# ShuangXieIrene/ssds.pytorch

Measured on AMD Instinct MI355X. Metric: images/sec (fwd+decode+NMS) SSD-MobileNetV2@512, higher is better.
Workload: dtype bf16

## Files before the change

ssds.pytorch_amd/csrc/ssdk_mbk.hip:

```cpp
#include "ssdk_common.h"
#include "ssdk_flow_common.h"
#include "ssdk_scan.h"

namespace ssdk {

struct MbkParams {
  const u16* x;
  u16* y;
  const unsigned char* img;
  int N, H, W, Ho, Wo, Cin, Chid, Cout, residual;
  int pairs, halves;
  unsigned items;
  unsigned long long* dbg;
  unsigned wave_mask, pair_mask;
};

template <int KS, int NW, int NCHW, int NFO>
struct MbkGeo {
  static constexpr int NP = (NCHW + 1) / 2;
  static constexpr int PAIR_KB = 2 * KS + NFO;
  static constexpr int MISC_KB = (NCHW * 384 + 1023) / 1024;
  static constexpr int m_be = 0, m_wd = NCHW * 64, m_bd = NCHW * (64 + 288);
  static constexpr int SPB_KB = 2;
  static_assert(NFO * 128 <= SPB_KB * 1024, "projection BN block");
  __host__ __device__ static size_t weights(int halves) { return (size_t)halves * NW * NP * PAIR_KB * 1024; }
  __host__ __device__ static size_t misc_off(int halves) { return weights(halves); }
  __host__ __device__ static size_t spb_off(int halves) { return misc_off(halves) + (size_t)NW * MISC_KB * 1024; }
  __host__ __device__ static size_t bytes(int halves) { return spb_off(halves) + (size_t)halves * SPB_KB * 1024; }
};

template <int S, int NS>
struct MbkItem {
  static constexpr int NXS = NS * S;
  static constexpr int NR = S + 3;
};

template <int S, int NS, int KS, int NW, int NCHW, int NFO>
struct MbkLds {
  using G = MbkGeo<KS, NW, NCHW, NFO>;
  using I = MbkItem<S, NS>;
  static constexpr int FT = 2 * NS * NFO;
  static constexpr int XF = FT % 5 == 0 ? 5 : (FT % 8 == 0 ? 8 : 4);
  static_assert(FT % XF == 0, "exchange rounds");
  static constexpr int xt = 0;
  static constexpr int misc = xt + I::NR * I::NXS * KS * 1024;
  static constexpr int spb = misc + NW * G::MISC_KB * 1024;
  static constexpr int xch = spb + G::SPB_KB * 1024;
  static constexpr int bytes = xch + NW * XF * 1024;
};

__device__ __forceinline__ void mbk_mfma_guard() {
  __builtin_amdgcn_sched_barrier(0);
  asm volatile("s_nop 15\n\ts_nop 3" ::: "memory");
  __builtin_amdgcn_sched_barrier(0);
}
__device__ __forceinline__ void mbk_valu_guard() {
  __builtin_amdgcn_sched_barrier(0);
  asm volatile("s_nop 3" ::: "memory");
  __builtin_amdgcn_sched_barrier(0);
}
__device__ __forceinline__ u32 fl_from_left2(u32 cur, u32 prev) {
  const int old = __builtin_amdgcn_update_dpp(0, (int)prev, 0x121, 0xf, 0xf, true);
  return (u32)__builtin_amdgcn_update_dpp(old, (int)cur, 0x111, 0xf, 0xf, false);
}
__device__ __forceinline__ u32 fl_from_right2(u32 cur, u32 next) {
  const int old = __builtin_amdgcn_update_dpp(0, (int)next, 0x12f, 0xf, 0xf, true);
  return (u32)__builtin_amdgcn_update_dpp(old, (int)cur, 0x101, 0xf, 0xf, false);
}

template <int DT, int S, int NS, int KS, int NW, int NCHW, int NFO, bool DBG = false>
__global__ __launch_bounds__(64 * NW, 2) void mbk_kernel(const MbkParams p) {
  using L = MbkLds<S, NS, KS, NW, NCHW, NFO>;
  using G = MbkGeo<KS, NW, NCHW, NFO>;
  using I = MbkItem<S, NS>;
  constexpr int NR = I::NR, NXS = I::NXS, NE = NR * NXS;
  constexpr int XF = L::XF, FT = L::FT, NP = G::NP, PAIR_KB = G::PAIR_KB;
  constexpr int NO = 2 * NS;
  constexpr bool ODD = (NCHW & 1) != 0;
  constexpr int ROUNDS = FT / XF;
  extern __shared__ __attribute__((aligned(16))) unsigned char smem[];
  const u32 tid = threadIdx.x, lane = tid & 63u;
  const u32 fr = lane & 15u, fg = lane >> 4;
  const int wv = __builtin_amdgcn_readfirstlane((int)(tid >> 6));
  const int Cin = p.Cin, Cout = p.Cout, H = p.H, W = p.W, Ho = p.Ho, Wo = p.Wo;

  const u32 item = blockIdx.x;
  const int half = (int)(item % (u32)p.halves);
  const u32 rem = item / (u32)p.halves;
  const int n = (int)(rem / (u32)p.pairs), rp = (int)(rem % (u32)p.pairs);
  const int oy0 = 2 * rp;
  const int iy0 = S * oy0 - 1;
  const int co_base = half * 16 * NFO;
  const u16* ximg = p.x + (size_t)n * H * W * Cin;
  const bool stamp = p.dbg != nullptr && blockIdx.x == 0 && tid == 0;
  if (stamp) p.dbg[0] = __builtin_readcyclecounter();

  const u32x4* wimg = reinterpret_cast<const u32x4*>(p.img + ((size_t)(half * NW + wv) * NP) * ((size_t)PAIR_KB * 1024)) + lane;
  u32x4 wa[KS], wb[KS];
#pragma unroll
  for (int ks = 0; ks < KS; ++ks) {
    wa[ks] = wimg[(size_t)ks * 64];
    wb[ks] = wimg[(size_t)(KS + ks) * 64];
  }

  for (int e = wv; e < NE; e += NW) {
    const int r = e / NXS, xs = e % NXS;
    int iy = iy0 + r;
    iy = iy < 0 ? 0 : (iy > H - 1 ? H - 1 : iy);
    const int col = S == 1 ? 16 * xs + (int)fr : 2 * (16 * (xs >> 1) + (int)fr) + (xs & 1);
    const u16* src = ximg + ((size_t)iy * W + col) * Cin + fg * 8;
#pragma unroll
    for (int ks = 0; ks < KS; ++ks)
      __builtin_amdgcn_global_load_lds((glb_u8*)(src + ks * 32), (lds_u8*)(smem + L::xt + (e * KS + ks) * 1024), 16, 0, 0);
  }
  {
    const unsigned char* src = p.img + G::misc_off(p.halves) + (size_t)wv * (G::MISC_KB * 1024) + lane * 16;
#pragma unroll
    for (int k = 0; k < G::MISC_KB; ++k)
      __builtin_amdgcn_global_load_lds((glb_u8*)(src + k * 1024), (lds_u8*)(smem + L::misc + (wv * G::MISC_KB + k) * 1024), 16, 0, 0);
  }
  if (wv == 0) {
    const unsigned char* src = p.img + G::spb_off(p.halves) + (size_t)half * (G::SPB_KB * 1024) + lane * 16;
#pragma unroll
    for (int k = 0; k < G::SPB_KB; ++k)
      __builtin_amdgcn_global_load_lds((glb_u8*)(src + k * 1024), (lds_u8*)(smem + L::spb + k * 1024), 16, 0, 0);
  }
  asm volatile("s_waitcnt vmcnt(0)" ::: "memory");
  __syncthreads();
  if (stamp) p.dbg[1] = __builtin_readcyclecounter();

  fl_f2 hi[NR];
#pragma unroll
  for (int r = 0; r < NR; ++r) {
    const float k = ((unsigned)(iy0 + r) < (unsigned)H) ? kFlSixth : 0.f;
    hi[r] = fl_f2{k, k};
  }

  f32x4 yacc[NO][NFO];
#pragma unroll
  for (int o = 0; o < NO; ++o)
#pragma unroll
    for (int f = 0; f < NFO; ++f) yacc[o][f] = f32x4{0.f, 0.f, 0.f, 0.f};

  const unsigned char* xt = smem + L::xt + lane * 16;
  const unsigned char* mc = smem + L::misc + wv * (G::MISC_KB * 1024);

  auto chunk = [&](int c, const u32x4 (&w)[KS], u32 (&dout)[NO][2]) {
    const f32x4 bv = *reinterpret_cast<const f32x4*>(mc + G::m_be + (c * 4 + (int)fg) * 16);
    f32x4 e[NE];
#pragma unroll
    for (int i = 0; i < NE; ++i) e[i] = bv;
#pragma unroll
    for (int ks = 0; ks < KS; ++ks) {
      u32x4 xf[NE];
#pragma unroll
      for (int i = 0; i < NE; ++i) xf[i] = *reinterpret_cast<const u32x4*>(xt + (i * KS + ks) * 1024);
#pragma unroll
      for (int i = 0; i < NE; ++i) e[i] = fl_mfma<DT>(w[ks], xf[i], e[i]);
    }
    uint2 wt[9];
#pragma unroll
    for (int t = 0; t < 9; ++t) wt[t] = *reinterpret_cast<const uint2*>(mc + G::m_wd + ((c * 9 + t) * 4 + (int)fg) * 8);
    const uint2 bdi = *reinterpret_cast<const uint2*>(mc + G::m_bd + (c * 4 + (int)fg) * 8);
    mbk_mfma_guard();
    u32 ew[NR][NXS][2];
#pragma unroll
    for (int r = 0; r < NR; ++r)
#pragma unroll
      for (int xs = 0; xs < NXS; ++xs) {
        ew[r][xs][0] = fl_unit_pack(e[r * NXS + xs][0], e[r * NXS + xs][1], hi[r]);
        ew[r][xs][1] = fl_unit_pack(e[r * NXS + xs][2], e[r * NXS + xs][3], hi[r]);
      }
#pragma unroll
    for (int o = 0; o < 2; ++o)
#pragma unroll
      for (int j = 0; j < NS; ++j) {
        fl_h2 s[2] = {fl_as_h2(bdi.x), fl_as_h2(bdi.y)};
#pragma unroll
        for (int ky = 0; ky < 3; ++ky) {
          const int r = S * o + ky;
          const uint2 w0 = wt[ky * 3], w1 = wt[ky * 3 + 1], w2 = wt[ky * 3 + 2];
#pragma unroll
          for (int wd = 0; wd < 2; ++wd) {
            u32 tl, tc, tr;
            if constexpr (S == 1) {
              tc = ew[r][j][wd];
              tl = j == 0 ? fl_from_left(tc) : fl_from_left2(tc, ew[r][j > 0 ? j - 1 : 0][wd]);
              tr = j == NS - 1 ? fl_from_right(tc) : fl_from_right2(tc, ew[r][j < NS - 1 ? j + 1 : j][wd]);
            } else {
              const u32 odd = ew[r][2 * j + 1][wd];
              tc = ew[r][2 * j][wd];
              tl = j == 0 ? fl_from_left(odd) : fl_from_left2(odd, ew[r][j > 0 ? 2 * j - 1 : 1][wd]);
              tr = odd;
            }
            const u32 ww0 = wd ? w0.y : w0.x, ww1 = wd ? w1.y : w1.x, ww2 = wd ? w2.y : w2.x;
            s[wd] = __builtin_elementwise_fma(fl_as_h2(tl), fl_as_h2(ww0), s[wd]);
            s[wd] = __builtin_elementwise_fma(fl_as_h2(tc), fl_as_h2(ww1), s[wd]);
            if (ky == 2) s[wd] = fl_fma_clamp01(fl_as_h2(tr), fl_as_h2(ww2), s[wd]);
            else s[wd] = __builtin_elementwise_fma(fl_as_h2(tr), fl_as_h2(ww2), s[wd]);
          }
        }
        dout[o * NS + j][0] = fl_as_u32(s[0]);
        dout[o * NS + j][1] = fl_as_u32(s[1]);
      }
  };

  constexpr int FH = NFO / 2;
  for (int t = 0; t < NP; ++t) {
    const u32x4* wp = wimg + (size_t)t * (PAIR_KB * 64);
    const bool last = t == NP - 1;
    const u32x4* wn = wimg + (size_t)(last ? t : t + 1) * (PAIR_KB * 64);
    u32 d0[NO][2], d1[NO][2];
    u32x4 wf0[FH], wf1[NFO - FH];
#pragma unroll
    for (int f = 0; f < FH; ++f) wf0[f] = wp[(size_t)(2 * KS + f) * 64];
    chunk(2 * t, wa, d0);
    __builtin_amdgcn_sched_barrier(0);
    u32x4 na[KS];
#pragma unroll
    for (int ks = 0; ks < KS; ++ks) na[ks] = wn[(size_t)ks * 64];
#pragma unroll
    for (int f = FH; f < NFO; ++f) wf1[f - FH] = wp[(size_t)(2 * KS + f) * 64];
    if (!(ODD && last)) {
      chunk(2 * t + 1, wb, d1);
    } else {
#pragma unroll
      for (int o = 0; o < NO; ++o) d1[o][0] = d1[o][1] = 0u;
    }
    __builtin_amdgcn_sched_barrier(0);
    u32x4 nb[KS];
#pragma unroll
    for (int ks = 0; ks < KS; ++ks) nb[ks] = wn[(size_t)(KS + ks) * 64];
    u32x4 db[NO];
#pragma unroll
    for (int o = 0; o < NO; ++o) db[o] = u32x4{d0[o][0], d0[o][1], d1[o][0], d1[o][1]};
    if constexpr (DBG) {
      if (!((p.pair_mask >> t) & 1u) || !((p.wave_mask >> wv) & 1u)) {
#pragma unroll
        for (int o = 0; o < NO; ++o) db[o] = u32x4{0u, 0u, 0u, 0u};
      }
    }
    mbk_valu_guard();
#pragma unroll
    for (int f = 0; f < NFO; ++f)
#pragma unroll
      for (int o = 0; o < NO; ++o)
        yacc[o][f] = fl_mfma<SSDK_F16>(f < FH ? wf0[f < FH ? f : 0] : wf1[f >= FH ? f - FH : 0], db[o], yacc[o][f]);
    __builtin_amdgcn_sched_barrier(0);
#pragma unroll
    for (int ks = 0; ks < KS; ++ks) {
      wa[ks] = na[ks];
      wb[ks] = nb[ks];
    }
  }
  if (stamp) p.dbg[2] = __builtin_readcyclecounter();

  unsigned char* xb = smem + L::xch;
  const unsigned char* spb = smem + L::spb;
  constexpr int GPW = (XF + NW - 1) / NW;
  uint2 resv[ROUNDS][GPW];
#pragma unroll
  for (int R = 0; R < ROUNDS; ++R)
#pragma unroll
    for (int gg = 0; gg < GPW; ++gg) {
      const int g = wv + gg * NW, q = R * XF + g, oj = q / NFO, f = q % NFO;
      const int oy = oy0 + oj / NS, ox = 16 * (oj % NS) + (int)fr, co = co_base + f * 16 + (int)fg * 4;
      resv[R][gg] = make_uint2(0u, 0u);
      if (S == 1 && p.residual && g < XF && oy < Ho && co < Cout)
        resv[R][gg] = *reinterpret_cast<const uint2*>(ximg + ((size_t)oy * W + ox) * Cin + co);
    }
#pragma unroll
  for (int R = 0; R < ROUNDS; ++R) {
#pragma unroll
    for (int g = 0; g < XF; ++g) {
      const int q = R * XF + g, oj = q / NFO, f = q % NFO;
      *reinterpret_cast<f32x4*>(xb + ((wv * XF + g) * 64 + (int)lane) * 16) = yacc[oj][f];
    }
    __syncthreads();
#pragma unroll
    for (int gg = 0; gg < GPW; ++gg) {
      const int g = wv + gg * NW;
      if (g < XF) {
        const int q = R * XF + g, oj = q / NFO, f = q % NFO;
        f32x4 y = *reinterpret_cast<const f32x4*>(xb + ((0 * XF + g) * 64 + (int)lane) * 16);
#pragma unroll
        for (int w2 = 1; w2 < NW; ++w2) {
          const f32x4 t2 = *reinterpret_cast<const f32x4*>(xb + ((w2 * XF + g) * 64 + (int)lane) * 16);
          y = y + t2;
        }
        const int oy = oy0 + oj / NS, ox = 16 * (oj % NS) + (int)fr;
        const int co = co_base + f * 16 + (int)fg * 4;
        if (oy < Ho && co < Cout) {
          const f32x4 spv = *reinterpret_cast<const f32x4*>(spb + (f * 4 + (int)fg) * 32);
          const f32x4 bpv = *reinterpret_cast<const f32x4*>(spb + (f * 4 + (int)fg) * 32 + 16);
          u32 h01 = fl_pack2<DT>(fmaf(y[0], spv[0], bpv[0]), fmaf(y[1], spv[1], bpv[1]));
          u32 h23 = fl_pack2<DT>(fmaf(y[2], spv[2], bpv[2]), fmaf(y[3], spv[3], bpv[3]));
          if (S == 1 && p.residual) {
            const uint2 xr = resv[R][gg];
            h01 = fl_pack2<DT>(fl_from16<DT>(h01 & 0xffffu) + fl_from16<DT>(xr.x & 0xffffu), fl_from16<DT>(h01 >> 16) + fl_from16<DT>(xr.x >> 16));
            h23 = fl_pack2<DT>(fl_from16<DT>(h23 & 0xffffu) + fl_from16<DT>(xr.y & 0xffffu), fl_from16<DT>(h23 >> 16) + fl_from16<DT>(xr.y >> 16));
          }
          u16* yrow = p.y + (((size_t)n * Ho + oy) * Wo + ox) * Cout;
          *reinterpret_cast<uint2*>(yrow + co) = make_uint2(h01, h23);
        }
      }
    }
    if (R + 1 < ROUNDS) __syncthreads();
  }
  if (stamp) p.dbg[3] = __builtin_readcyclecounter();
}

template <int DT, int S, int NS, int KS, int NW, int NCHW, int NFO, bool DBG = false>
static void mbk_launch(const MbkParams& p, hipStream_t stream) {
  constexpr int lds = MbkLds<S, NS, KS, NW, NCHW, NFO>::bytes;
  static_assert(lds <= 160 * 1024, "LDS");
  (void)hipFuncSetAttribute(reinterpret_cast<const void*>(&mbk_kernel<DT, S, NS, KS, NW, NCHW, NFO, DBG>),
                            hipFuncAttributeMaxDynamicSharedMemorySize, lds);
  hipLaunchKernelGGL((mbk_kernel<DT, S, NS, KS, NW, NCHW, NFO, DBG>), dim3(p.items), dim3(64 * NW), lds, stream, p);
}

constexpr int kMbkNW = 4;
struct MbkInst {
  int s, ns, ks, nchw, nfo;
};
static const MbkInst kMbkInst[] = {{1, 1, 5, 15, 10}, {2, 1, 3, 9, 10}, {1, 2, 2, 6, 4}, {1, 2, 2, 6, 6}, {1, 2, 3, 9, 6},
                                   {2, 2, 1, 3, 4}, {1, 4, 1, 3, 2}};

static int mbk_find(int stride, int Wo, int Cin, int Chid, int Cout, int nw, int* halves) {
  if (nw != kMbkNW || Cin % 32 || Chid % 16 || Cout % 16 || Wo % 16) return -1;
  const int ks = Cin / 32, nch = Chid / 16, nchw = (nch + nw - 1) / nw, ns = Wo / 16;
  for (int i = 0; i < (int)(sizeof(kMbkInst) / sizeof(kMbkInst[0])); ++i) {
    const MbkInst& k = kMbkInst[i];
    if (k.s == stride && k.ns == ns && k.ks == ks && k.nchw == nchw && Cout % (16 * k.nfo) == 0) {
      if (halves) *halves = Cout / (16 * k.nfo);
      return i;
    }
  }
  return -1;
}

static size_t mbk_bytes(int inst, int halves) {
  switch (inst) {
    case 0: return MbkGeo<5, kMbkNW, 15, 10>::bytes(halves);
    case 1: return MbkGeo<3, kMbkNW, 9, 10>::bytes(halves);
    case 2: return MbkGeo<2, kMbkNW, 6, 4>::bytes(halves);
    case 3: return MbkGeo<2, kMbkNW, 6, 6>::bytes(halves);
    case 4: return MbkGeo<3, kMbkNW, 9, 6>::bytes(halves);
    case 5: return MbkGeo<1, kMbkNW, 3, 4>::bytes(halves);
    case 6: return MbkGeo<1, kMbkNW, 3, 2>::bytes(halves);
  }
  return 0;
}

template <int DT>
static void mbk_dispatch(const MbkParams& p, int inst, hipStream_t stream) {
  const bool dbg = p.wave_mask != ~0u || p.pair_mask != ~0u;
  switch (inst) {
    case 0: dbg ? mbk_launch<DT, 1, 1, 5, kMbkNW, 15, 10, true>(p, stream) : mbk_launch<DT, 1, 1, 5, kMbkNW, 15, 10>(p, stream); break;
    case 1: mbk_launch<DT, 2, 1, 3, kMbkNW, 9, 10>(p, stream); break;
    case 2: mbk_launch<DT, 1, 2, 2, kMbkNW, 6, 4>(p, stream); break;
    case 3: mbk_launch<DT, 1, 2, 2, kMbkNW, 6, 6>(p, stream); break;
    case 4: mbk_launch<DT, 1, 2, 3, kMbkNW, 9, 6>(p, stream); break;
    case 5: mbk_launch<DT, 2, 2, 1, kMbkNW, 3, 4>(p, stream); break;
    case 6: mbk_launch<DT, 1, 4, 1, kMbkNW, 3, 2>(p, stream); break;
  }
}

int launch_mbk(const ssdk_mbconv_desc* d, hipStream_t stream) {
  static const int env = getenv("SSDK_MBK") ? atoi(getenv("SSDK_MBK")) : 1;
  const int variant = d->variant;
  if ((!env && variant != 3) || (variant != 0 && variant != 3)) return 1;
  if (d->stem || !d->w_image || d->image_nw < 1 || (d->stride != 1 && d->stride != 2)) return 1;
  const int Ho = (d->H + 2 - 3) / d->stride + 1, Wo = (d->W + 2 - 3) / d->stride + 1;
  if (d->W != Wo * d->stride) return 1;
  int halves = 0;
  const int inst = mbk_find(d->stride, Wo, d->Cin, d->Chid, d->Cout, d->image_nw, &halves);
  if (inst < 0 || (size_t)d->w_image_bytes < mbk_bytes(inst, halves) || ((uintptr_t)d->w_image & 15)) return 1;
  if (env != 1 && variant != 3 && !((env >> (inst + 1)) & 1)) return 1;
  const int pairs = (Ho + 1) / 2;
  const long items = (long)halves * d->N * pairs;
  constexpr int env_min = 256;
  if (items < env_min && variant != 3) return 1;
  MbkParams p;
  p.x = (const u16*)d->x;
  p.y = (u16*)d->y;
  p.img = (const unsigned char*)d->w_image;
  p.N = d->N;
  p.H = d->H;
  p.W = d->W;
  p.Ho = Ho;
  p.Wo = Wo;
  p.Cin = d->Cin;
  p.Chid = d->Chid;
  p.Cout = d->Cout;
  p.residual = d->residual;
  p.pairs = pairs;
  p.halves = halves;
  p.items = (unsigned)items;
  p.dbg = nullptr;
  p.wave_mask = p.pair_mask = ~0u;
  if (const char* m = getenv("SSDK_MBK_MASKS")) {
    unsigned a = ~0u, b = ~0u;
    if (sscanf(m, "%x,%x", &a, &b) == 2) {
      p.wave_mask = a;
      p.pair_mask = b;
    }
  }
  static const int env_dbg = getenv("SSDK_MB_DBG") ? atoi(getenv("SSDK_MB_DBG")) : 0;
  static unsigned long long* dbg_dev = nullptr;
  if (env_dbg) {
    if (!dbg_dev) (void)hipMalloc(&dbg_dev, 8 * sizeof(unsigned long long));
    p.dbg = dbg_dev;
  }
  if (d->dtype == SSDK_BF16) mbk_dispatch<SSDK_BF16>(p, inst, stream);
  else mbk_dispatch<SSDK_F16>(p, inst, stream);
  if (env_dbg) {
    unsigned long long h[4];
    (void)hipStreamSynchronize(stream);
    (void)hipMemcpy(h, dbg_dev, sizeof(h), hipMemcpyDeviceToHost);
    fprintf(stderr, "[mbk dbg] Cin=%d Chid=%d Cout=%d s=%d W=%d items=%ld : setup %llu loop %llu exchange %llu\n", d->Cin, d->Chid,
            d->Cout, d->stride, d->W, items, h[1] - h[0], h[2] - h[1], h[3] - h[2]);
  }
  return 0;
}

}

extern "C" size_t ssdk_mbk_image_bytes(int Cin, int Chid, int Cout, int stride, int Wo, int nw, int* nfo) {
  int halves = 0;
  const int inst = ssdk::mbk_find(stride, Wo, Cin, Chid, Cout, nw, &halves);
  if (inst < 0) return 0;
  if (nfo) *nfo = ssdk::kMbkInst[inst].nfo;
  return ssdk::mbk_bytes(inst, halves);
}
```

Baseline: 64660.

## Process four output rows per block for the first MBConv instance

Generalises the fused MBConv kernel from two output rows per work item to a template parameter R, and sets R=4 for instance 0 (stride 1, KS=5, 15 hidden chunks per wave). Each block now loads a taller input halo (3R+... rows) once, so the weight image and halo rows are amortised over more outputs and fewer blocks are launched. For R=4 the input tile is also preloaded into registers once instead of re-read from LDS for every hidden chunk. In exchange, register pressure rises sharply, occupancy drops to one block per SIMD via launch bounds, and the number of blocks is halved, which could hurt latency hiding and load balance.

```diff
diff --git a/ssds.pytorch_amd/csrc/ssdk_mbk.hip b/ssds.pytorch_amd/csrc/ssdk_mbk.hip
--- a/ssds.pytorch_amd/csrc/ssdk_mbk.hip
+++ b/ssds.pytorch_amd/csrc/ssdk_mbk.hip
@@ -9,7 +9,7 @@
   u16* y;
   const unsigned char* img;
   int N, H, W, Ho, Wo, Cin, Chid, Cout, residual;
-  int pairs, halves;
+  int groups, halves;
   unsigned items;
   unsigned long long* dbg;
   unsigned wave_mask, pair_mask;
@@ -29,18 +29,19 @@
   __host__ __device__ static size_t bytes(int halves) { return spb_off(halves) + (size_t)halves * SPB_KB * 1024; }
 };
 
-template <int S, int NS>
+template <int S, int NS, int R>
 struct MbkItem {
+  static_assert(R == 2 || R == 4, "rows per item");
   static constexpr int NXS = NS * S;
-  static constexpr int NR = S + 3;
+  static constexpr int NR = S * (R - 1) + 3;
 };
 
-template <int S, int NS, int KS, int NW, int NCHW, int NFO>
+template <int S, int NS, int KS, int NW, int NCHW, int NFO, int R>
 struct MbkLds {
   using G = MbkGeo<KS, NW, NCHW, NFO>;
-  using I = MbkItem<S, NS>;
-  static constexpr int FT = 2 * NS * NFO;
-  static constexpr int XF = FT % 5 == 0 ? 5 : (FT % 8 == 0 ? 8 : 4);
+  using I = MbkItem<S, NS, R>;
+  static constexpr int FT = R * NS * NFO;
+  static constexpr int XF = FT % 8 == 0 ? 8 : (FT % 5 == 0 ? 5 : 4);
   static_assert(FT % XF == 0, "exchange rounds");
   static constexpr int xt = 0;
   static constexpr int misc = xt + I::NR * I::NXS * KS * 1024;
@@ -68,14 +69,14 @@
   return (u32)__builtin_amdgcn_update_dpp(old, (int)cur, 0x101, 0xf, 0xf, false);
 }
 
-template <int DT, int S, int NS, int KS, int NW, int NCHW, int NFO, bool DBG = false>
-__global__ __launch_bounds__(64 * NW, 2) void mbk_kernel(const MbkParams p) {
-  using L = MbkLds<S, NS, KS, NW, NCHW, NFO>;
+template <int DT, int S, int NS, int KS, int NW, int NCHW, int NFO, int R, bool DBG = false>
+__global__ __launch_bounds__(64 * NW, R == 2 ? 2 : 1) void mbk_kernel(const MbkParams p) {
+  using L = MbkLds<S, NS, KS, NW, NCHW, NFO, R>;
   using G = MbkGeo<KS, NW, NCHW, NFO>;
-  using I = MbkItem<S, NS>;
+  using I = MbkItem<S, NS, R>;
   constexpr int NR = I::NR, NXS = I::NXS, NE = NR * NXS;
   constexpr int XF = L::XF, FT = L::FT, NP = G::NP, PAIR_KB = G::PAIR_KB;
-  constexpr int NO = 2 * NS;
+  constexpr int NO = R * NS;
   constexpr bool ODD = (NCHW & 1) != 0;
   constexpr int ROUNDS = FT / XF;
   extern __shared__ __attribute__((aligned(16))) unsigned char smem[];
@@ -87,8 +88,8 @@
   const u32 item = blockIdx.x;
   const int half = (int)(item % (u32)p.halves);
   const u32 rem = item / (u32)p.halves;
-  const int n = (int)(rem / (u32)p.pairs), rp = (int)(rem % (u32)p.pairs);
-  const int oy0 = 2 * rp;
+  const int n = (int)(rem / (u32)p.groups), rg = (int)(rem % (u32)p.groups);
+  const int oy0 = R * rg;
   const int iy0 = S * oy0 - 1;
   const int co_base = half * 16 * NFO;
   const u16* ximg = p.x + (size_t)n * H * W * Cin;
@@ -144,6 +145,12 @@
 
   const unsigned char* xt = smem + L::xt + lane * 16;
   const unsigned char* mc = smem + L::misc + wv * (G::MISC_KB * 1024);
+  constexpr int NXR = R == 4 ? NE * KS : 1;
+  u32x4 xr[NXR];
+  if constexpr (R == 4) {
+#pragma unroll
+    for (int i = 0; i < NE * KS; ++i) xr[i] = *reinterpret_cast<const u32x4*>(xt + i * 1024);
+  }
 
   auto chunk = [&](int c, const u32x4 (&w)[KS], u32 (&dout)[NO][2]) {
     const f32x4 bv = *reinterpret_cast<const f32x4*>(mc + G::m_be + (c * 4 + (int)fg) * 16);
@@ -154,7 +161,8 @@
     for (int ks = 0; ks < KS; ++ks) {
       u32x4 xf[NE];
 #pragma unroll
-      for (int i = 0; i < NE; ++i) xf[i] = *reinterpret_cast<const u32x4*>(xt + (i * KS + ks) * 1024);
+      for (int i = 0; i < NE; ++i)
+        xf[i] = R == 4 ? xr[R == 4 ? i * KS + ks : 0] : *reinterpret_cast<const u32x4*>(xt + (i * KS + ks) * 1024);
 #pragma unroll
       for (int i = 0; i < NE; ++i) e[i] = fl_mfma<DT>(w[ks], xf[i], e[i]);
     }
@@ -172,7 +180,7 @@
         ew[r][xs][1] = fl_unit_pack(e[r * NXS + xs][2], e[r * NXS + xs][3], hi[r]);
       }
 #pragma unroll
-    for (int o = 0; o < 2; ++o)
+    for (int o = 0; o < R; ++o)
 #pragma unroll
       for (int j = 0; j < NS; ++j) {
         fl_h2 s[2] = {fl_as_h2(bdi.x), fl_as_h2(bdi.y)};
@@ -260,20 +268,20 @@
   constexpr int GPW = (XF + NW - 1) / NW;
   uint2 resv[ROUNDS][GPW];
 #pragma unroll
-  for (int R = 0; R < ROUNDS; ++R)
+  for (int rd = 0; rd < ROUNDS; ++rd)
 #pragma unroll
     for (int gg = 0; gg < GPW; ++gg) {
-      const int g = wv + gg * NW, q = R * XF + g, oj = q / NFO, f = q % NFO;
+      const int g = wv + gg * NW, q = rd * XF + g, oj = q / NFO, f = q % NFO;
       const int oy = oy0 + oj / NS, ox = 16 * (oj % NS) + (int)fr, co = co_base + f * 16 + (int)fg * 4;
-      resv[R][gg] = make_uint2(0u, 0u);
+      resv[rd][gg] = make_uint2(0u, 0u);
       if (S == 1 && p.residual && g < XF && oy < Ho && co < Cout)
-        resv[R][gg] = *reinterpret_cast<const uint2*>(ximg + ((size_t)oy * W + ox) * Cin + co);
-    }
-#pragma unroll
-  for (int R = 0; R < ROUNDS; ++R) {
+        resv[rd][gg] = *reinterpret_cast<const uint2*>(ximg + ((size_t)oy * W + ox) * Cin + co);
+    }
+#pragma unroll
+  for (int rd = 0; rd < ROUNDS; ++rd) {
 #pragma unroll
     for (int g = 0; g < XF; ++g) {
-      const int q = R * XF + g, oj = q / NFO, f = q % NFO;
+      const int q = rd * XF + g, oj = q / NFO, f = q % NFO;
       *reinterpret_cast<f32x4*>(xb + ((wv * XF + g) * 64 + (int)lane) * 16) = yacc[oj][f];
     }
     __syncthreads();
@@ -281,7 +289,7 @@
     for (int gg = 0; gg < GPW; ++gg) {
       const int g = wv + gg * NW;
       if (g < XF) {
-        const int q = R * XF + g, oj = q / NFO, f = q % NFO;
+        const int q = rd * XF + g, oj = q / NFO, f = q % NFO;
         f32x4 y = *reinterpret_cast<const f32x4*>(xb + ((0 * XF + g) * 64 + (int)lane) * 16);
 #pragma unroll
         for (int w2 = 1; w2 < NW; ++w2) {
@@ -296,7 +304,7 @@
           u32 h01 = fl_pack2<DT>(fmaf(y[0], spv[0], bpv[0]), fmaf(y[1], spv[1], bpv[1]));
           u32 h23 = fl_pack2<DT>(fmaf(y[2], spv[2], bpv[2]), fmaf(y[3], spv[3], bpv[3]));
           if (S == 1 && p.residual) {
-            const uint2 xr = resv[R][gg];
+            const uint2 xr = resv[rd][gg];
             h01 = fl_pack2<DT>(fl_from16<DT>(h01 & 0xffffu) + fl_from16<DT>(xr.x & 0xffffu), fl_from16<DT>(h01 >> 16) + fl_from16<DT>(xr.x >> 16));
             h23 = fl_pack2<DT>(fl_from16<DT>(h23 & 0xffffu) + fl_from16<DT>(xr.y & 0xffffu), fl_from16<DT>(h23 >> 16) + fl_from16<DT>(xr.y >> 16));
           }
@@ -305,26 +313,28 @@
         }
       }
     }
-    if (R + 1 < ROUNDS) __syncthreads();
+    if (rd + 1 < ROUNDS) __syncthreads();
   }
   if (stamp) p.dbg[3] = __builtin_readcyclecounter();
 }
 
-template <int DT, int S, int NS, int KS, int NW, int NCHW, int NFO, bool DBG = false>
+template <int DT, int S, int NS, int KS, int NW, int NCHW, int NFO, int R, bool DBG = false>
 static void mbk_launch(const MbkParams& p, hipStream_t stream) {
-  constexpr int lds = MbkLds<S, NS, KS, NW, NCHW, NFO>::bytes;
+  constexpr int lds = MbkLds<S, NS, KS, NW, NCHW, NFO, R>::bytes;
   static_assert(lds <= 160 * 1024, "LDS");
-  (void)hipFuncSetAttribute(reinterpret_cast<const void*>(&mbk_kernel<DT, S, NS, KS, NW, NCHW, NFO, DBG>),
+  (void)hipFuncSetAttribute(reinterpret_cast<const void*>(&mbk_kernel<DT, S, NS, KS, NW, NCHW, NFO, R, DBG>),
                             hipFuncAttributeMaxDynamicSharedMemorySize, lds);
-  hipLaunchKernelGGL((mbk_kernel<DT, S, NS, KS, NW, NCHW, NFO, DBG>), dim3(p.items), dim3(64 * NW), lds, stream, p);
+  hipLaunchKernelGGL((mbk_kernel<DT, S, NS, KS, NW, NCHW, NFO, R, DBG>), dim3(p.items), dim3(64 * NW), lds, stream, p);
 }
 
 constexpr int kMbkNW = 4;
+constexpr int kMbkR[7] = {4, 2, 2, 2, 2, 2, 2};
 struct MbkInst {
-  int s, ns, ks, nchw, nfo;
+  int s, ns, ks, nchw, nfo, r;
 };
-static const MbkInst kMbkInst[] = {{1, 1, 5, 15, 10}, {2, 1, 3, 9, 10}, {1, 2, 2, 6, 4}, {1, 2, 2, 6, 6}, {1, 2, 3, 9, 6},
-                                   {2, 2, 1, 3, 4}, {1, 4, 1, 3, 2}};
+static const MbkInst kMbkInst[] = {{1, 1, 5, 15, 10, kMbkR[0]}, {2, 1, 3, 9, 10, kMbkR[1]}, {1, 2, 2, 6, 4, kMbkR[2]},
+                                   {1, 2, 2, 6, 6, kMbkR[3]},   {1, 2, 3, 9, 6, kMbkR[4]},  {2, 2, 1, 3, 4, kMbkR[5]},
+                                   {1, 4, 1, 3, 2, kMbkR[6]}};
 
 static int mbk_find(int stride, int Wo, int Cin, int Chid, int Cout, int nw, int* halves) {
   if (nw != kMbkNW || Cin % 32 || Chid % 16 || Cout % 16 || Wo % 16) return -1;
@@ -356,13 +366,13 @@
 static void mbk_dispatch(const MbkParams& p, int inst, hipStream_t stream) {
   const bool dbg = p.wave_mask != ~0u || p.pair_mask != ~0u;
   switch (inst) {
-    case 0: dbg ? mbk_launch<DT, 1, 1, 5, kMbkNW, 15, 10, true>(p, stream) : mbk_launch<DT, 1, 1, 5, kMbkNW, 15, 10>(p, stream); break;
-    case 1: mbk_launch<DT, 2, 1, 3, kMbkNW, 9, 10>(p, stream); break;
-    case 2: mbk_launch<DT, 1, 2, 2, kMbkNW, 6, 4>(p, stream); break;
-    case 3: mbk_launch<DT, 1, 2, 2, kMbkNW, 6, 6>(p, stream); break;
-    case 4: mbk_launch<DT, 1, 2, 3, kMbkNW, 9, 6>(p, stream); break;
-    case 5: mbk_launch<DT, 2, 2, 1, kMbkNW, 3, 4>(p, stream); break;
-    case 6: mbk_launch<DT, 1, 4, 1, kMbkNW, 3, 2>(p, stream); break;
+    case 0: dbg ? mbk_launch<DT, 1, 1, 5, kMbkNW, 15, 10, kMbkR[0], true>(p, stream) : mbk_launch<DT, 1, 1, 5, kMbkNW, 15, 10, kMbkR[0]>(p, stream); break;
+    case 1: mbk_launch<DT, 2, 1, 3, kMbkNW, 9, 10, kMbkR[1]>(p, stream); break;
+    case 2: mbk_launch<DT, 1, 2, 2, kMbkNW, 6, 4, kMbkR[2]>(p, stream); break;
+    case 3: mbk_launch<DT, 1, 2, 2, kMbkNW, 6, 6, kMbkR[3]>(p, stream); break;
+    case 4: mbk_launch<DT, 1, 2, 3, kMbkNW, 9, 6, kMbkR[4]>(p, stream); break;
+    case 5: mbk_launch<DT, 2, 2, 1, kMbkNW, 3, 4, kMbkR[5]>(p, stream); break;
+    case 6: mbk_launch<DT, 1, 4, 1, kMbkNW, 3, 2, kMbkR[6]>(p, stream); break;
   }
 }
 
@@ -377,10 +387,12 @@
   const int inst = mbk_find(d->stride, Wo, d->Cin, d->Chid, d->Cout, d->image_nw, &halves);
   if (inst < 0 || (size_t)d->w_image_bytes < mbk_bytes(inst, halves) || ((uintptr_t)d->w_image & 15)) return 1;
   if (env != 1 && variant != 3 && !((env >> (inst + 1)) & 1)) return 1;
-  const int pairs = (Ho + 1) / 2;
-  const long items = (long)halves * d->N * pairs;
-  constexpr int env_min = 256;
-  if (items < env_min && variant != 3) return 1;
+  const long rows = (long)halves * d->N * (2 * ((Ho + 1) / 2));
+  constexpr int env_min_rows = 512;
+  if (rows < env_min_rows && variant != 3) return 1;
+  const int R = kMbkInst[inst].r;
+  const int groups = (Ho + R - 1) / R;
+  const long items = (long)halves * d->N * groups;
   MbkParams p;
   p.x = (const u16*)d->x;
   p.y = (u16*)d->y;
@@ -394,7 +406,7 @@
   p.Chid = d->Chid;
   p.Cout = d->Cout;
   p.residual = d->residual;
-  p.pairs = pairs;
+  p.groups = groups;
   p.halves = halves;
   p.items = (unsigned)items;
   p.dbg = nullptr;
```

Result: no change. 65070 (median of 6 runs) (+0.6%).
